# igorauad/gr-dvbs2rx

Hardware: AMD Instinct MI355X
Metric: FECFRAMEs/sec (coded Gbit/s) @ 50 LDPC iters, QPSK 1/2 normal (higher is better)
Workload: dtype int8; 1 GPU; QPSK 1/2 normal FECFRAME (DVB_S2_TABLE_B4, N=64800), 50 LDPC iterations cap, batch=4096 frames per GPU, group G=32, input=noise; frames_per_gpu=4096, max_trials=50, group_size=32, parallelism=frames sharded over 1 GPU(s), no collective

## Files before the change

### gr-dvbs2rx_amd/csrc/ldpc_kernel.hpp

```cpp
#pragma once
#include <hip/hip_runtime.h>
#include <cstdint>
#include "demap_math.hpp"
#include "ldpc_launch.h"
#include "ldpc_prims.hpp"
#include "ldpc_node_plain.hpp"
#include "ldpc_node_packed.hpp"
#include "ldpc_node_hazard.hpp"

namespace dvbs2 {

#define DVBS2_DEG_CASE(D) case D: if constexpr (D >= 3 && D <= DMAX && D > DMAX - 8) { \
        { if (layer0) check_node<(D >= 3 ? D : 3), true, false, false, TC>(lds_all, ent, jj, lb, mw, nm); else { if constexpr (!kPure) check_node<(D >= 3 ? D : 3), false, false, false, TC>(lds_all, ent, jj, lb, mw, nm); } } } else DVBS2_NM_CLEAR break;
#define DVBS2_DEG_SWITCH switch (deg) { DVBS2_DEGREES_3_32(DVBS2_DEG_CASE) default: DVBS2_NM_CLEAR break; }

#define DVBS2_V2_CASE(D) case D: if constexpr (D >= 3 && D <= DMAX && D > DMAX - 8) { check_node_v2<(D >= 3 ? D : 3), DMAX, TC>(ent, jj + lb, mw, nm, prefetch); } else DVBS2_NM_CLEAR break;
#define DVBS2_V2_SWITCH switch (deg) { DVBS2_DEGREES_3_32(DVBS2_V2_CASE) default: DVBS2_NM_CLEAR break; }
#define DVBS2_NM_CLEAR { _Pragma("unroll") for (int w_ = 0; w_ < MW; w_++) nm[w_] = 0u; }

#define DVBS2_CHAIN_CASE(D) case D: if constexpr (D >= 4 && D <= DMAX && D > DMAX - 8) { check_node_chain_v2<(D >= 4 ? D : 4), DMAX, TC>(ent, jj, jj + lb, work, block, mw, nm, htab16, hb_ctr, hb_epoch, hb_lane); } break;
#define DVBS2_CHAIN_SWITCH switch (deg) { DVBS2_DEGREES_4_32(DVBS2_CHAIN_CASE) default: break; }

#define DVBS2_HAZ_NODE(D, NCV, ...) \
        check_node_hazard<D, NCV, HazardCfg<hz::two_level<HZ2>, hz::chain_ok<(MINW == 1)>, hz::class8<(DMAX <= 8)>, hz::tc<TC>, __VA_ARGS__>>( \
            lds_all, ent, jj, lb, work, block, block2, mw, nm, 0, nullptr, htab, hb_ctr, hb_epoch, hb_lane, hz_ph);
#define DVBS2_HAZ_CALL1(D, NCV, LRV, TLCV) { \
        if (layer0) DVBS2_HAZ_NODE(D, NCV, hz::layer0<true>, hz::low_reg<LRV>, hz::tlc<TLCV>) \
        else { if constexpr (!kPure) DVBS2_HAZ_NODE(D, NCV, hz::layer0<false>, hz::low_reg<LRV>, hz::tlc<TLCV>) } }
#define DVBS2_HAZ_CALL(D, NCV) { if constexpr (D - 2 >= NCV) { \
        if constexpr (kTlc<DMAX, HZ2> && !SOFT && MINW == 1 && (NCV == 4 || NCV == 8)) { if (block2 > 0 && htab != nullptr) DVBS2_HAZ_CALL1(D, NCV, (DMAX >= kTlcLowRegMinDmax), true) else DVBS2_HAZ_CALL1(D, NCV, false, false) } \
        else DVBS2_HAZ_CALL1(D, NCV, false, false) } }
#define DVBS2_HAZ_CASE(D) case D: if constexpr (D >= 4 && D <= DMAX && D > DMAX - 8) { \
        if (nc == 2) DVBS2_HAZ_CALL((D >= 4 ? D : 4), 2) else if (nc == 4) DVBS2_HAZ_CALL((D >= 4 ? D : 4), 4) else { if constexpr (HZ2 && DMAX <= kMaxHazard12Dmax) { if (nc == 8) DVBS2_HAZ_CALL((D >= 4 ? D : 4), 8) else DVBS2_HAZ_CALL((D >= 4 ? D : 4), 12) } else DVBS2_HAZ_CALL((D >= 4 ? D : 4), 8) } } break;
#define DVBS2_HAZP_CALL1(D, NCV, TLCV) { DVBS2_HAZ_NODE(D, NCV, hz::tlc<TLCV>, hz::packed_phases<true>, hz::dmaxv<DMAX>) }
#define DVBS2_HAZP_CALL(D, NCV) { if constexpr (D - 2 >= NCV) { \
        if constexpr (kTlc<DMAX, HZ2> && !SOFT && MINW == 1 && (NCV == 4 || NCV == 8)) { if (block2 > 0 && htab != nullptr) DVBS2_HAZP_CALL1(D, NCV, true) else DVBS2_HAZP_CALL1(D, NCV, false) } \
        else DVBS2_HAZP_CALL1(D, NCV, false) } }
#define DVBS2_HAZP_CASE(D) case D: if constexpr (D >= 4 && D <= DMAX && D > DMAX - 8) { \
        if (nc == 2) DVBS2_HAZP_CALL((D >= 4 ? D : 4), 2) else if (nc == 4) DVBS2_HAZP_CALL((D >= 4 ? D : 4), 4) else DVBS2_HAZP_CALL((D >= 4 ? D : 4), 8) } break;
#define DVBS2_HAZP_SWITCH switch (deg) { DVBS2_DEGREES_4_32(DVBS2_HAZP_CASE) default: break; }
#define DVBS2_HAZ_SWITCH switch (deg) { DVBS2_DEGREES_4_32(DVBS2_HAZ_CASE) default: break; }

__device__ __attribute__((noinline)) int syndrome_sign_vectors(const lds_byte_t* lds, lds_u32_t* sv, int N, int tid, bool tc )
{
    lds_byte_t* svb = reinterpret_cast<lds_byte_t*>(sv);
    int zero = 0;
#pragma unroll 2
    for (int blk = tid; blk < N / 8; blk += kHalf) {
        const v2u32 v = *reinterpret_cast<const lds_v2u_t*>(lds + 8 * blk);
        const uint32_t ob = tc ? 0u : 0x80808080u;
        const uint32_t xa = v.x ^ ob, xb = v.y ^ ob;
        zero |= (int)((((xa - 0x01010101u) & ~xa) | ((xb - 0x01010101u) & ~xb)) & 0x80808080u);
        const uint32_t na = (((xa & 0x80808080u) >> 7) * 0x01020408u) >> 24, nb = (((xb & 0x80808080u) >> 7) * 0x01020408u) >> 24;
        const int g = blk / 45;
        svb[g * (kSvWords * 4) + (blk - 45 * g)] = (uint8_t)((na & 0xfu) | ((nb & 0xfu) << 4));
    }
    return zero;
}

constexpr int kSoloThreads = 512;
static_assert(kCuSlots == 16 * 8 * 2 * 16, "the per-CU counter table (ldpc_layout.h) must hold every index hw_cu_index() can return: XCC x SE x SH x CU");
__device__ __forceinline__ uint32_t hw_cu_index()
{
    uint32_t hw, xcc;
    asm volatile("s_getreg_b32 %0, hwreg(HW_REG_HW_ID)" : "=s"(hw));
    asm volatile("s_getreg_b32 %0, hwreg(HW_REG_XCC_ID)" : "=s"(xcc));
    return ((((xcc & 0xfu) * 8u + ((hw >> 13) & 7u)) * 2u + ((hw >> 12) & 1u)) * 16u + ((hw >> 8) & 0xfu));
}

template <int DMAX, bool TIMING, int MINW = 1, bool V2 = false, bool SOLO = false, bool HZ2 = false, bool SOFT = false
          >
__global__ __launch_bounds__(SOLO ? kSoloThreads : kThreads, SOLO ? 4 : MINW) void ldpc_layered_kernel(
    const uint32_t* __restrict__ recs, const uint32_t* __restrict__ wrecs ,
    const int8_t* __restrict__ llr_in, uint8_t* __restrict__ state,
    uint32_t* __restrict__ msgs, int* __restrict__ iters, int* __restrict__ good, const int* __restrict__ target,
    int n_frames, int N, int K, int q, int cap, int stop_on_good ,
    unsigned long long* __restrict__ tdbg, int* __restrict__ cu_slots,
    const DemapFused dm )
{
    unsigned long long tm_bar = 0, tm_body = 0, tm_conf = 0, tm_synd = 0, tm_sweep = 0, tm_load = 0, tm_s1 = 0;
#define TSTAMP(x) do { if (TIMING) { x = __builtin_readcyclecounter(); } } while (0)
    unsigned long long tA = 0, tB = 0, tC = 0, tS0 = 0, tS1 = 0;
    const bool fresh = llr_in != nullptr || dm.mode != 0;
    if (!fresh) {
        const int fa = SOLO ? (int)blockIdx.x : 2 * (int)blockIdx.x, fb = SOLO ? fa : fa + 1;
        const bool ta = fa < n_frames && iters[fa] < target[fa];
        const bool tb = fb < n_frames && iters[fb] < target[fb];
        if (!ta && !tb) return;
    }
    TSTAMP(tA);
    extern __shared__ __attribute__((aligned(16))) uint8_t lds_all[];
    constexpr int RS = rec_stride(DMAX);
    constexpr int RSW = V2 ? 6 * rec_stride_wave(DMAX) : rec_stride(DMAX);
    constexpr int MW = DMAX / 4;
    constexpr bool kPure = V2 && v2_pure_class(DMAX);
    constexpr bool TC = V2 && DMAX <= kTcMaxDmax;
    constexpr uint32_t kObState = TC ? 0x80808080u : 0u;
    int solo_tid = (int)threadIdx.x;
    int solo_slot = -1, solo_pat = 0;
    if constexpr (SOLO) {
        volatile lds_i32_t* e = reinterpret_cast<volatile lds_i32_t*>((lds_byte_t*)lds_all);
        if (threadIdx.x < 8) e[threadIdx.x] = 0;
        __syncthreads();
        if (threadIdx.x == 0) {
            solo_slot = (int)hw_cu_index();
            int* w = cu_slots + solo_slot;
            int old = __hip_atomic_load(w, __ATOMIC_RELAXED, __HIP_MEMORY_SCOPE_AGENT), pat;
            do { pat = (old & 0xffff) <= (old >> 16) ? 0 : 1; }
            while (!__hip_atomic_compare_exchange_strong(w, &old, old + (pat ? 0x10000 : 1), __ATOMIC_RELAXED, __ATOMIC_RELAXED, __HIP_MEMORY_SCOPE_AGENT));
            e[5] = pat; e[6] = solo_slot;
        }
        __syncthreads();
        solo_pat = e[5]; solo_slot = e[6];
        int widx = -1;
        if ((threadIdx.x & 63) == 0) {
            uint32_t hw;
            asm volatile("s_getreg_b32 %0, hwreg(HW_REG_HW_ID)" : "=s"(hw));
            const int simd = (int)((hw >> 4) & 3u);
            const int rank = __hip_atomic_fetch_add(const_cast<lds_i32_t*>(e) + simd, 1, __ATOMIC_RELAXED, __HIP_MEMORY_SCOPE_WORKGROUP);
            const bool two = ((simd >> 1) & 1) == solo_pat;
            if (two || rank == 0) widx = __hip_atomic_fetch_add(const_cast<lds_i32_t*>(e) + 4, 1, __ATOMIC_RELAXED, __HIP_MEMORY_SCOPE_WORKGROUP);
        }
        widx = __builtin_amdgcn_readfirstlane(widx);
        __syncthreads();
        const int nworkers = e[4];
        if (nworkers != 6) widx = (int)(threadIdx.x >> 6) < 6 ? (int)(threadIdx.x >> 6) : -1;
        __syncthreads();
        if (widx < 0 || widx >= 6) return;
        solo_tid = widx * 64 + (int)(threadIdx.x & 63);
    }
    const int half = SOLO ? 0 : __builtin_amdgcn_readfirstlane(threadIdx.x >= kHalf ? 1 : 0);
    const int tid = SOLO ? solo_tid : (int)threadIdx.x - half * kHalf;
    const int lb_rel = half * (int)half_lds_bytes(N);
    const int lb = lb_rel + lds_address_of(lds_all);
    lds_byte_t* lds = (lds_byte_t*)lds_all + lb_rel;
    lds_u32_t* sv = reinterpret_cast<lds_u32_t*>(lds + N);
    volatile lds_i32_t* flags = reinterpret_cast<volatile lds_i32_t*>(sv + sv_area_words(N));
    volatile lds_i32_t* other_flags = reinterpret_cast<volatile lds_i32_t*>(
        (lds_byte_t*)lds_all + (1 - half) * (int)half_lds_bytes(N) + N + sv_area_words(N) * 4);
    const int f = SOLO ? (int)blockIdx.x : 2 * (int)blockIdx.x + half;
    const bool have_frame = f < n_frames;
    const int lane = tid & 63, wave = tid >> 6;
    const int wave_u = __builtin_amdgcn_readfirstlane(wave);
    const int NG = N / kM;
    const bool active = tid < kM;

    int it = 0, tgt = 0;
    bool finished = !have_frame;
    if (have_frame) {
        tgt = target ? target[f] : cap;
        if (fresh && dm.mode != 0) {
            auto put = [&](int n, int8_t v) {
                int idx = n;
                if (n >= K) { const int r = n - K, jq = r / q; idx = K + kM * (r - jq * q) + jq; }
                lds[idx] = (uint8_t)v ^ (TC ? 0x00u : 0x80u);
            };
            const float N0 = dm.n0[dm.n0_count > 1 ? f : 0];
            const float2* src = reinterpret_cast<const float2*>(dm.syms) + (size_t)f * dm.n_syms;
            if (dm.mode == 1) {
                const float scalar = qpsk_scalar(N0);
                for (int sidx = tid; sidx < dm.n_syms; sidx += kHalf) {
                    const float2 v = src[sidx];
                    put(2 * sidx, qpsk_llr(v.x, scalar)); put(2 * sidx + 1, qpsk_llr(v.y, scalar));
                }
            } else {
                const float dp = psk8_dist_prec(N0);
                for (int sidx = tid; sidx < dm.n_syms; sidx += kHalf) {
                    const float2 v = src[sidx];
                    int8_t b0, b1, b2;
                    psk8_llr(v.x, v.y, dm.rr, dm.ri, dp, b0, b1, b2);
                    put(dm.ra0 + sidx, b0); put(dm.ra1 + sidx, b1); put(dm.ra2 + sidx, b2);
                }
            }
        } else if (fresh) {
            const uint2* src = reinterpret_cast<const uint2*>(llr_in + (size_t)f * N);
            for (int c = tid; c < N / 8; c += kHalf) {
                uint2 v = src[c];
                if constexpr (!TC) { v.x ^= 0x80808080u; v.y ^= 0x80808080u; }
                const int n = 8 * c;
                if (n < K) *reinterpret_cast<lds_v2u_t*>(lds + n) = (v2u32){ v.x, v.y };
                else {
                    int r = n - K;
                    int jq = r / q, iq = r - jq * q;
#pragma unroll
                    for (int b = 0; b < 8; b++) {
                        lds[K + kM * iq + jq] = (uint8_t)((b < 4 ? v.x >> (8 * b) : v.y >> (8 * (b - 4))) & 0xffu);
                        if (++iq == q) { iq = 0; ++jq; }
                    }
                }
            }
        } else {
            it = iters[f];
            if (it >= tgt) finished = true;
            else {
                const uint2* src = reinterpret_cast<const uint2*>(state + (size_t)f * N);
                for (int c = tid; c < N / 8; c += kHalf) { const uint2 v = src[c]; *reinterpret_cast<lds_v2u_t*>(lds + 8 * c) = (v2u32){ v.x ^ kObState, v.y ^ kObState }; }
            }
        }
    }
    const bool untouched = finished;
    if (tid == 0) { flags[0] = 0; flags[2] = 0; flags[3] = 0; flags[1] = finished ? 1 : 0; flags[4] = 0; }
    constexpr bool soft_bar = SOFT;
    volatile lds_i32_t* hb_ctr = soft_bar ? flags + 4 : nullptr;
    int hb_epoch = 0;
    const int hb_lane = lane;
    __syncthreads();
    TSTAMP(tB); tm_load = tB - tA;

    uint32_t* msg_base = msgs + (size_t)(have_frame ? f : 0) * q * MW * kMsgStride;
    const __amdgpu_buffer_rsrc_t mrs = __builtin_amdgcn_make_buffer_rsrc(msg_base, 0, q * MW * kMsgStride * 4, 0x00020000);
    constexpr int kLayerBytes = MW * kMsgStride * 4;
#define MSG_LD(soff, w, r4) __builtin_amdgcn_raw_buffer_load_b32(mrs, (r4), (soff) + (w) * (kMsgStride * 4), 0)
#define MSG_ST(v, soff, w, r4) __builtin_amdgcn_raw_buffer_store_b32((v), mrs, (r4), (soff) + (w) * (kMsgStride * 4), 0)
    auto msg_load = [&](uint32_t* dst, int soff, int r4) {
#pragma unroll
        for (int w = 0; w < MW; w++) dst[w] = MSG_LD(soff, w, r4);
    };
    auto msg_store = [&](const uint32_t* src, int soff, int r4) {
#pragma unroll
        for (int w = 0; w < MW; w++) MSG_ST(src[w], soff, w, r4);
    };
    auto take_msgs = [&](uint32_t* mw, uint32_t* pre, bool zero, uint32_t zero_word, int next, int r4) {
#pragma unroll
        for (int w = 0; w < MW; w++) mw[w] = pre[w];
        if (zero) {
            asm volatile("" ::: "memory");
#pragma unroll
            for (int w = 0; w < MW; w++) mw[w] = zero_word;
        } else msg_load(pre, next, r4);
    };
    bool is_good = false;

    for (;;) {
        TSTAMP(tS0);
        const bool need_synd = !finished && ((stop_on_good & 1) || it >= tgt);
        if (need_synd && active) {
            const int i0 = it % q;
            const uint32_t* rec = recs + (size_t)i0 * RS;
            const int deg = (int)(rec[0] & 0xffu) + 2;
            uint32_t x = 0, z = 0;
            constexpr bool kPretestChunk = DMAX != 16 && !(DMAX == 32 && SOFT);
            if constexpr (kPretestChunk) {
            for (int k0 = 0; k0 < deg; k0 += 4) {
                uint32_t e[8], v[4];
#pragma unroll
                for (int u = 0; u < 8; u++) e[u] = rec[4 + 2 * k0 + u];
#pragma unroll
                for (int u = 0; u < 4; u++) {
                    const int a0 = tid + (int)e[2 * u] - ((uint32_t)tid < e[2 * u + 1] ? 0 : kM);
                    v[u] = (uint32_t)lds[k0 + u < deg ? a0 : tid];
                }
#pragma unroll
                for (int u = 0; u < 4; u++) {
                    uint32_t w = v[u] ^ (TC ? 0x80u : 0x00u);
                    if (i0 == 0 && k0 + u == deg - 1 && tid == 0) w = 0x81u;
                    if (k0 + u < deg) { x ^= w; z |= (w == 0x80u); }
                }
            }
            } else
            for (int k = 0; k < deg; k++) {
                const int a0 = tid + (int)rec[4 + 2 * k] - ((uint32_t)tid < rec[5 + 2 * k] ? 0 : kM);
                uint32_t v = (uint32_t)lds[a0] ^ (TC ? 0x80u : 0x00u);
                if (i0 == 0 && k == deg - 1 && tid == 0) v = 0x81u;
                x ^= v;
                z |= (v == 0x80u);
            }
            const int bad_pre = (int)((((x >> 7) ^ (uint32_t)deg) & 1u) | z);
            if (__ballot(bad_pre) != 0 && lane == 0) flags[2] = 1;
        }
        lds_barrier();
        const bool need_full = need_synd && flags[2] == 0;
        if (tid == 0) flags[3] = need_full ? 1 : 0;
        lds_barrier();
        const bool full_any = flags[3] != 0 || (!soft_bar && !SOLO && other_flags[3] != 0);
        if (full_any) {
        if (need_full) {
            {
                const int zero = syndrome_sign_vectors(lds, sv, N, tid, TC);
                if (__ballot(zero != 0) != 0 && lane == 0) flags[0] = 1;
            }
        }
        TSTAMP(tC); tm_s1 += tC - tS0;
        lds_barrier();
        if (need_full && tid < NG) {
            lds_u32_t* p = sv + tid * kSvWords;
            const uint32_t w0 = p[0], w1 = p[1];
            p[11] = (p[11] & 0xffu) | (w0 << 8);
            p[12] = (w0 >> 24) | (w1 << 8);
        }
        lds_barrier();
        if (need_full) {
            int bad = 0;
            for (int item = tid; item < q * 12; item += kHalf) {
                const int i = item / 12, w = item - 12 * i;
                const uint32_t* rec = recs + (size_t)i * RS;
                const int deg = (int)(rec[0] & 0xffu) + 2;
                uint32_t e0[DMAX], e1[DMAX];
#pragma unroll
                for (int k = 0; k < DMAX; k++) { e0[k] = rec[4 + 2 * k]; e1[k] = rec[5 + 2 * k]; }
                uint32_t acc = 0;
#pragma unroll
                for (int k = 0; k < DMAX; k++) {
                    if (k < deg) {
                        const int rot = kM - (int)e1[k];
                        const int g360 = (int)e0[k] - rot;
                        const int t0 = wrap360(32 * w + rot);
                        const lds_u32_t* p = sv + (g360 / kM) * kSvWords + (t0 >> 5);
                        uint32_t x = __funnelshift_r(p[0], p[1], t0 & 31);
                        if (i == 0 && k == deg - 1 && w == 0) x &= ~1u;
                        acc ^= x;
                    }
                }
                if (w == 11) acc &= 0xffu;
                bad |= acc != 0;
            }
            if (__ballot(bad) != 0 && lane == 0) flags[0] = 1;
        }
        lds_barrier();
        }
        if (need_synd) is_good = need_full && flags[0] == 0;
        const bool gs = (stop_on_good & 5) == 5;
        if (!finished && (it >= tgt || (!gs && (stop_on_good & 1) && is_good))) finished = true;
        lds_barrier();
        if (wave_u == 0) {
            int fin = finished ? 1 : 0;
            if (gs && !finished) {
                const uint32_t* hd = recs - kRecHeaderWords;
                const int* iters0 = reinterpret_cast<const int*>(((unsigned long long)hd[1] << 32) | hd[0]);
                int* status = reinterpret_cast<int*>(((unsigned long long)hd[3] << 32) | hd[2]);
                const int G = (int)hd[4];
                const int g = f / G;
                fin = group_decide(status + (iters - iters0) + g * G, min(G, n_frames - g * G), f - g * G, it, is_good, lane, (int)hd[5]) != 0;
            }
            if (tid == 0) { flags[0] = 0; flags[2] = 0; flags[1] = fin; }
        }
        lds_only_barrier();
        if (gs) finished = flags[1] != 0;
        TSTAMP(tS1); tm_synd += tS1 - tS0;
        if (finished && (soft_bar || SOLO || other_flags[1])) break;

        const bool work = __builtin_amdgcn_readfirstlane(finished ? 0 : 1) != 0;
        const int row = tid < kM ? tid : kM - 1;
        const int row4 = row * 4;
        const bool zero_msgs = __builtin_amdgcn_readfirstlane(it) == 0;
        unsigned long long* const hz_ph = (TIMING && tdbg && f == 0 && (tid == 0 || tid == 320)) ? tdbg + (size_t)n_frames * 48 + 256 + (tid ? 16 : 0) : nullptr;
        uint32_t pre[MW];
        constexpr bool kWaitStore = !SOFT;
        if (work) {
#pragma unroll
            for (int w = 0; w < MW; w++) {
                pre[w] = zero_msgs ? 0x80808080u : MSG_LD(0, w, row4);
            }
        }
        constexpr int kPfSmallMaxDmax = 8;
        constexpr int PF = DMAX <= kPfSmallMaxDmax ? 1 : 2 * DMAX;
        const uint32_t* wr = V2 ? wrecs + (size_t)wave_u * rec_stride_wave(DMAX) : recs;
        uint32_t nhdr = wr[0], nw1 = wr[1];
        uint32_t nent[2 * DMAX];
#pragma unroll
        for (int k = 0; k < 2 * DMAX; k += PF) nent[k] = wr[4 + k];
        DVBS2_WAIT_VM0();
        asm volatile("" : "+s"(nhdr), "+s"(nw1), "+s"(nent[0]));
        for (int i = 0; i < q; i++) {
            const uint32_t hdr = nhdr;
            uint32_t ent[2 * DMAX];
#pragma unroll
            for (int k = 0; k < 2 * DMAX; k++) ent[k] = (PF <= 2 * DMAX - 1 && k % PF == 0) ? nent[k] : wr[(size_t)i * RSW + 4 + k];
            const int inext = i + 1 < q ? i + 1 : 0;
            const uint32_t* nrec = wr + (size_t)inext * RSW;
            auto prefetch = [&](uint32_t after) {
                const uint32_t* p = nrec; (void)after;
                nhdr = p[0];
                if constexpr (PF <= 2 * DMAX - 1) {
#pragma unroll
                    for (int k = 0; k < 2 * DMAX; k += PF) nent[k] = p[4 + k];
                }
            };
            constexpr int kPabMaxDmax = 8;
            constexpr bool kPab = DMAX <= kPabMaxDmax;
            if constexpr (!kPab) prefetch(0u);
            const int deg = (int)(hdr & 0xffu) + 2;
            const int nc = (int)((hdr >> 8) & 0xfu);
            lds_u32_t* htab = ((hdr >> 12) & 1u) ? sv : nullptr;
            const int block = (int)(hdr >> 16);
            int block2 = 0;
            if constexpr (HZ2 || (kTlc<DMAX, HZ2> && !SOFT && MINW == 1)) { if (block < kM) block2 = (int)wr[(size_t)i * RSW + 2]; }
            const bool layer0 = (i == 0);
            const int mso = i * kLayerBytes;
            TSTAMP(tA);
            if (hdr & 0x8000u) lds_barrier();
            if constexpr (kPab) { asm volatile("" ::: "memory"); prefetch(0u); }
            TSTAMP(tB); tm_bar += tB - tA;
            if (block >= kM) {
                if (work) {
                    const int jj = row;
                    const bool v2 = V2 && ((hdr >> 13) & 1u);
                    uint32_t mw[MW], nm[MW];
                    take_msgs(mw, pre, zero_msgs, v2 ? 0u : 0x80808080u, inext * kLayerBytes, row4);
                    if constexpr (V2) { if (v2) { DVBS2_V2_SWITCH } else DVBS2_DEG_SWITCH } else DVBS2_DEG_SWITCH
                    DVBS2_WAIT_VM0();
                    msg_store(nm, mso, row4);
                }
                TSTAMP(tC); tm_body += tC - tB;
                if (TIMING && tdbg && f == 0 && tid == 0) tdbg[(size_t)n_frames * 48 + i] += tC - tA;
            } else {
                if (nc != kHazardWalk) {
                    const int jj = row;
                    const bool hv2 = V2 && ((hdr >> 13) & 1u);
                    uint32_t mw[MW], nm[MW];
#pragma unroll
                    for (int w = 0; w < MW; w++) mw[w] = (work && !zero_msgs) ? pre[w] : (hv2 ? 0u : 0x80808080u);
                    if (work && i + 1 < q && !zero_msgs) msg_load(pre, mso + kLayerBytes, row4);
                    const bool hvp = V2 && v2p_class(DMAX) && ((hdr >> 14) & 1u);
                    if constexpr (V2 && DMAX <= 16) {
                        if (hv2) {
                            lds_u32_t* htab16 = lds_align16<lds_u32_t>(sv);
                            DVBS2_CHAIN_SWITCH
                        } else DVBS2_HAZ_SWITCH
                    } else if constexpr (V2 && v2p_class(DMAX)) { if (hvp) { DVBS2_HAZP_SWITCH } else DVBS2_HAZ_SWITCH }
                    else DVBS2_HAZ_SWITCH
                    DVBS2_WAIT_VM0();
                    if (work) msg_store(nm, mso, row4);
                } else {
                    if (!finished && wave == 0) {
                        const int chunk = block < 64 ? block : 64;
                        for (int start = 0; start < kM; start += chunk) {
                            const int jj = start + lane;
                            if (lane < chunk && jj < kM) {
                                uint32_t mw[MW], nm[MW];
#pragma unroll
                                for (int w = 0; w < MW; w++) mw[w] = zero_msgs ? 0x80808080u : MSG_LD(mso, w, jj * 4);
                                DVBS2_DEG_SWITCH
#pragma unroll
                                for (int w = 0; w < MW; w++) MSG_ST(nm[w], mso, w, jj * 4);
                            }
                        }
                    }
                    lds_barrier();
                    if (work && i + 1 < q && !zero_msgs) msg_load(pre, mso + kLayerBytes, row4);
                    DVBS2_WAIT_VM0();
                }
                TSTAMP(tC); tm_conf += tC - tB;
                if (TIMING && tdbg && f == 0 && tid == 0) tdbg[(size_t)n_frames * 48 + i] += tC - tA;
            }
        }
        TSTAMP(tA);
        lds_barrier();
        TSTAMP(tB); tm_bar += tB - tA; tm_sweep += tB - tS1;
        if (!finished) it++;
    }
    if (TIMING && tdbg && lane == 0 && have_frame) {
        unsigned long long* o = tdbg + ((size_t)f * 6 + wave) * 8;
        o[0] = tm_load; o[1] = tm_synd; o[2] = tm_sweep; o[3] = tm_bar; o[4] = tm_body; o[5] = tm_conf; o[6] = (unsigned long long)it; o[7] = tm_s1;
    }

    if (have_frame && !untouched) {
        if (tid == 0) { iters[f] = it; good[f] = is_good ? 1 : 0; }
        uint2* dst = reinterpret_cast<uint2*>(state + (size_t)f * N);
        for (int c = tid; c < N / 8; c += kHalf) { const v2u32 v = *reinterpret_cast<const lds_v2u_t*>(lds + 8 * c); dst[c] = make_uint2(v.x ^ kObState, v.y ^ kObState); }
    }
    if constexpr (SOLO) {
        if (tid == 0) __hip_atomic_fetch_add(cu_slots + solo_slot, solo_pat ? -0x10000 : -1, __ATOMIC_RELAXED, __HIP_MEMORY_SCOPE_AGENT);
    }
}

}
```

Baseline: 143,600 frames/s.

## Add run loop for consecutive same-degree packed layers with double-buffered records

For small-degree V2 codes, runs of consecutive packed, non-hazard layers of the same degree are processed in a dedicated loop. The degree switch is resolved once per run, and records and messages are ping-ponged between two register sets so the next layer's record and messages load while the current check node computes. The goal is to cut per-layer dispatch and header decoding and to overlap loads better. In exchange, the generic path now uses the plain degree switch for V2 when kRun holds, which could change code size and register pressure.

```diff
diff --git a/gr-dvbs2rx_amd/csrc/ldpc_kernel.hpp b/gr-dvbs2rx_amd/csrc/ldpc_kernel.hpp
--- a/gr-dvbs2rx_amd/csrc/ldpc_kernel.hpp
+++ b/gr-dvbs2rx_amd/csrc/ldpc_kernel.hpp
@@ -17,6 +17,7 @@
 #define DVBS2_V2_CASE(D) case D: if constexpr (D >= 3 && D <= DMAX && D > DMAX - 8) { check_node_v2<(D >= 3 ? D : 3), DMAX, TC>(ent, jj + lb, mw, nm, prefetch); } else DVBS2_NM_CLEAR break;
 #define DVBS2_V2_SWITCH switch (deg) { DVBS2_DEGREES_3_32(DVBS2_V2_CASE) default: DVBS2_NM_CLEAR break; }
 #define DVBS2_NM_CLEAR { _Pragma("unroll") for (int w_ = 0; w_ < MW; w_++) nm[w_] = 0u; }
+#define DVBS2_RUN_CASE(D) case D - 2: if constexpr (D >= 3 && D <= DMAX && D > DMAX - 8) { run(std::integral_constant<int, (D >= 3 ? D : 3)>{}); } break;
 
 #define DVBS2_CHAIN_CASE(D) case D: if constexpr (D >= 4 && D <= DMAX && D > DMAX - 8) { check_node_chain_v2<(D >= 4 ? D : 4), DMAX, TC>(ent, jj, jj + lb, work, block, mw, nm, htab16, hb_ctr, hb_epoch, hb_lane); } break;
 #define DVBS2_CHAIN_SWITCH switch (deg) { DVBS2_DEGREES_4_32(DVBS2_CHAIN_CASE) default: break; }
@@ -352,8 +353,10 @@
                 pre[w] = zero_msgs ? 0x80808080u : MSG_LD(0, w, row4);
             }
         }
+        constexpr bool kRun = V2 && DMAX <= 8;
         constexpr int kPfSmallMaxDmax = 8;
         constexpr int PF = DMAX <= kPfSmallMaxDmax ? 1 : 2 * DMAX;
+        static_assert(!kRun || PF == 1, "the run loop takes over whole records fetched ahead into scalar registers");
         const uint32_t* wr = V2 ? wrecs + (size_t)wave_u * rec_stride_wave(DMAX) : recs;
         uint32_t nhdr = wr[0], nw1 = wr[1];
         uint32_t nent[2 * DMAX];
@@ -362,6 +365,63 @@
         DVBS2_WAIT_VM0();
         asm volatile("" : "+s"(nhdr), "+s"(nw1), "+s"(nent[0]));
         for (int i = 0; i < q; i++) {
+            if constexpr (kRun) {
+                if (work && (nhdr & kRecPacked) && (nhdr >> kRecBlockShift) >= (uint32_t)kM) {
+                    auto run = [&](auto degc) {
+                        constexpr int D = decltype(degc)::value;
+                        uint32_t ha = nhdr, hb = 0u, ea[2 * DMAX], eb[2 * DMAX], pb[MW];
+#pragma unroll
+                        for (int k = 0; k < 2 * DMAX; k++) { ea[k] = nent[k]; eb[k] = 0u; }
+#pragma unroll
+                        for (int w = 0; w < MW; w++) pb[w] = 0u;
+                        bool more;
+#define DVBS2_RUN_TRIP(H, E, P, NH, NE, NP) { \
+                            const int inext = i + 1 < q ? i + 1 : 0; \
+                            const uint32_t* nrec = wr + (size_t)inext * RSW; \
+                            TSTAMP(tA); \
+                            if (H & (1u << kRecSyncShift)) lds_barrier(); \
+                            asm volatile("" ::: "memory"); \
+                            NH = nrec[0]; \
+                            _Pragma("unroll") for (int k = 0; k < 2 * DMAX; k++) NE[k] = nrec[4 + k]; \
+                            TSTAMP(tB); tm_bar += tB - tA; \
+                            uint32_t mw[MW], nm[MW]; \
+                            _Pragma("unroll") for (int w = 0; w < MW; w++) mw[w] = P[w]; \
+                            if (zero_msgs) { \
+                                asm volatile("" ::: "memory"); \
+                                _Pragma("unroll") for (int w = 0; w < MW; w++) mw[w] = 0u; \
+                            } else msg_load(NP, inext * kLayerBytes, row4); \
+                            check_node_v2<D, DMAX, TC>(E, row + lb, mw, nm, 0); \
+                            DVBS2_WAIT_VM0(); \
+                            msg_store(nm, i * kLayerBytes, row4); \
+                            TSTAMP(tC); tm_body += tC - tB; \
+                            if (TIMING && tdbg && f == 0 && tid == 0) tdbg[(size_t)n_frames * 48 + i] += tC - tA; \
+                            more = inext != 0 && ((NH ^ H) & (0xffu | kRecPacked)) == 0u && (NH >> kRecBlockShift) >= (uint32_t)kM; }
+                        for (;;) {
+                            DVBS2_RUN_TRIP(ha, ea, pre, hb, eb, pb)
+                            if (!more) {
+                                nhdr = hb;
+#pragma unroll
+                                for (int k = 0; k < 2 * DMAX; k++) nent[k] = eb[k];
+#pragma unroll
+                                for (int w = 0; w < MW; w++) pre[w] = pb[w];
+                                break;
+                            }
+                            i++;
+                            DVBS2_RUN_TRIP(hb, eb, pb, ha, ea, pre)
+                            if (!more) {
+                                nhdr = ha;
+#pragma unroll
+                                for (int k = 0; k < 2 * DMAX; k++) nent[k] = ea[k];
+                                break;
+                            }
+                            i++;
+                        }
+#undef DVBS2_RUN_TRIP
+                    };
+                    switch (nhdr & 0xffu) { DVBS2_DEGREES_3_7(DVBS2_RUN_CASE) DVBS2_RUN_CASE(8) default: break; }
+                    continue;
+                }
+            }
             const uint32_t hdr = nhdr;
             uint32_t ent[2 * DMAX];
 #pragma unroll
@@ -397,7 +457,7 @@
                     const bool v2 = V2 && ((hdr >> 13) & 1u);
                     uint32_t mw[MW], nm[MW];
                     take_msgs(mw, pre, zero_msgs, v2 ? 0u : 0x80808080u, inext * kLayerBytes, row4);
-                    if constexpr (V2) { if (v2) { DVBS2_V2_SWITCH } else DVBS2_DEG_SWITCH } else DVBS2_DEG_SWITCH
+                    if constexpr (V2 && !kRun) { if (v2) { DVBS2_V2_SWITCH } else DVBS2_DEG_SWITCH } else DVBS2_DEG_SWITCH
                     DVBS2_WAIT_VM0();
                     msg_store(nm, mso, row4);
                 }
```

After: 146,100 frames/s, median of 6. +1.7%, better.
